# Westlake-AI/SemiReward

Measured on AMD Instinct MI355X. Metric: unlabeled images/sec/node (FlexMatch+SR, ViT-S CIFAR-100), higher is better.
Workload: dtype bf16

## Files before the change

include/srhip.h:

```cpp
#ifndef SRHIP_H
#define SRHIP_H

#ifdef __cplusplus
extern "C" {
#endif

enum {
  SRHIP_EPI_BF16 = 0,
  SRHIP_EPI_GELU_BF16 = 1,
  SRHIP_EPI_RESID_F32 = 2,
  SRHIP_EPI_DGELU_BF16 = 3,
  SRHIP_EPI_F32 = 4
};
int srhip_gemm_nt(int epilogue, const void* A, int lda, const void* B, int ldb, void* C, int ldc, int M, int N, int K,
                  const float* bias, const float* row_scale, int rows_per_sample, const void* aux_in, void* aux_out,
                  int ldaux, float alpha, float beta, void* stream);
#define SRHIP_GEMM_PLAN_TILE128 0
#define SRHIP_GEMM_PLAN_SMALL64 1
#define SRHIP_GEMM_PLAN_BIG256 2
#define SRHIP_GEMM_PLAN_BIG128 3
#define SRHIP_GEMM_PLAN_BIG2WG 4
#define SRHIP_GEMM_PLAN_PP256 5
int srhip_gemm_nt_plan(int epilogue, int M, int N, int K, float beta);
int srhip_gemm_nt_planned(int epilogue, const void* A, int lda, const void* B, int ldb, void* C, int ldc, int M, int N, int K,
// ... 32 lines not shown
} srhip_slab_desc;
int srhip_slab_reduce_f32(const srhip_slab_desc* desc_dev, int n, int total_blocks, void* stream);
int srhip_gemm_tn_grouped_pp_f32(const srhip_group_tn_desc* desc_dev, int n_problems, int total_tiles, float alpha, float beta,
                                 void* stream);

int srhip_attn_fwd(const void* qkv, void* out, float* lse, int B, int N, int H, float scale, void* stream);
int srhip_attn_bwd(const void* qkv, const void* out, const void* d_out, const float* lse, void* dqkv, float* delta_ws,
                   int B, int N, int H, float scale, void* stream);

int srhip_attn_masked_fwd(const void* qkv, void* out, float* lse, const int* key_len, int B, int N, int H, float scale,
                          unsigned drop_key, unsigned drop_thresh, float drop_scale, void* stream);
int srhip_attn_masked_bwd(const void* qkv, const void* out, const void* d_out, const float* lse, void* dqkv, float* delta_ws,
                          const int* key_len, int B, int N, int H, float scale, unsigned drop_key, unsigned drop_thresh,
                          float drop_scale, void* stream);

int srhip_layernorm_fwd(const float* x, const float* gamma, const float* beta, float eps, void* out, float* mean,
                        float* rstd, int M, int D, void* stream);
int srhip_layernorm_bwd(const void* dy, const float* x, const float* mean, const float* rstd, const float* gamma,
                        float* dx, float* dgamma, float* dbeta, int M, int D, void* stream);
int srhip_layernorm_bwd_cast(const void* dy, const float* x, const float* mean, const float* rstd, const float* gamma, float* dx, float* dgamma,
                             float* dbeta, void* out_bf16, const float* row_scale, int rows_per_sample, int M, int D, void* stream);
int srhip_layernorm_bwd_part(const void* dy, const float* x, const float* mean, const float* rstd, const float* gamma, float* dx, float* part,
                             int n_rep, void* out_bf16, const float* row_scale, int rows_per_sample, int M, int D, void* stream);
typedef struct srhip_ln_reduce_desc { float* dgamma; float* dbeta; } srhip_ln_reduce_desc;
int srhip_ln_grad_reduce(const srhip_ln_reduce_desc* desc_dev, float* part, int n_ln, int n_rep, int D, void* stream);
typedef struct srhip_dw_tail {
  const srhip_ln_reduce_desc* ln_desc; float* ln_part;
  const float* dlogits; const float* feat; float* dWh; float* dbh;
  const float* dx; const float* img; const int* img_index; float* dpos; float* dcls; float* pe_ws;
  int n_ln, n_rep, C, B, D, in_chans, HW, ps;
} srhip_dw_tail;
int srhip_gemm_tn_grouped_tail_f32(const srhip_group_tn_desc* desc_dev, int n_problems, int total_tiles, float alpha, float beta,
                                   const srhip_dw_tail* tail, void* stream);
int srhip_patch_embed_bwd_fold(const float* ws, float* dWp, float* dbp, int B, int C, int HW, int ps, int D, void* stream);

int srhip_mlp_fused(const float* x, float* x_out, const float* ln_gamma, const float* ln_beta, float eps, const void* W1,
                    const float* b1, const void* W2, const float* b2, const float* row_scale, int rows_per_sample, int save_rows,
                    void* save_ln2, void* save_pre, void* save_h, float* save_mean, float* save_rstd, int M, int D, int Hd,
                    void* stream);
int srhip_gelu_eval(const float* x, float* y_erf, float* y_poly, int n, void* stream);
int srhip_mlp_fused_proj(const float* x, float* x_out, const void* ao, const void* Wp, const float* bp, const float* row_scale1,
                         int ao_scaled, const float* ln_gamma, const float* ln_beta, float eps, const void* W1, const float* b1, const void* W2,
                         const float* b2, const float* row_scale2, int rows_per_sample, void* ln_next, const float* next_gamma,
                         const float* next_beta, int M, int D, int Hd, void* stream);
int srhip_mlp_fused_proj_strided(const float* x, float* x_out, const void* ao, const void* Wp, const float* bp, const float* row_scale1,
                                 int ao_scaled, const float* ln_gamma, const float* ln_beta, float eps, const void* W1, const float* b1,
                                 const void* W2, const float* b2, const float* row_scale2, int rows_per_sample, void* ln_next,
                                 const float* next_gamma, const float* next_beta, int M, int D, int Hd, int row_pitch, void* stream);

int srhip_attn_block_supported(int N, int D, int H);
int srhip_attn_block_fused(const void* xn_bf16, const void* Wqkv, const float* bqkv, const void* qkv_extra, void* out, const float* out_scale,
                           int B, int N, int D, int H, float scale, void* stream);

int srhip_patch_embed_fwd(const float* img, const int* img_index, const float* Wp, const float* bp, const float* cls,
                          const float* pos, float* x, int B, int C, int HW, int ps, int D, void* stream);
int srhip_patch_embed_bwd(const float* dx, const float* img, const int* img_index, float* dWp, float* dbp, float* dcls,
                          float* dpos, int B, int C, int HW, int ps, int D, void* stream);
long srhip_patch_embed_bwd_ws_floats(int B, int C, int HW, int ps, int D);
int srhip_patch_embed_bwd_ws(const float* dx, const float* img, const int* img_index, float* dWp, float* dbp, float* dcls,
                             float* dpos, float* ws, int B, int C, int HW, int ps, int D, void* stream);

int srhip_patch_im2col(const float* img, const int* img_index, void* out, int B, int C, int HW, int ps, void* stream);
int srhip_patch_assemble(const float* tok, const float* bp, const float* cls, const float* pos, float* x, int B, int Np, int D,
                         void* stream);
int srhip_patch_grad_operands(const float* dx, void* dx_tok_bf16, float* dpos, float* dcls, int B, int Np, int D, void* stream);

// ... 284 lines not shown
```

semireward_amd/_lib.py:

```python
import ctypes
import os
from ctypes import c_double, c_float, c_int, c_long, c_longlong, c_uint, c_ulonglong, c_void_p

import torch

HERE = os.path.dirname(os.path.abspath(__file__))
LIB_PATH = os.path.join(HERE, "libsrhip.so")

EPI_BF16, EPI_GELU_BF16, EPI_RESID_F32, EPI_DGELU_BF16, EPI_F32 = range(5)
X3_EPI_F32, X3_EPI_GELU_F32, X3_EPI_RESID_F32 = range(3)
X3B_NT, X3B_NN = range(2)
X3B_EPI_F32, X3B_EPI_ACC, X3B_EPI_DGELU, X3B_EPI_GELU_PRE = range(4)
REDUCE_NONE, REDUCE_MEAN, REDUCE_SUM = range(3)
SCORE_FIXED, SCORE_FLEX, SCORE_FREE, SCORE_SOFT = range(4)

P, I, F, L, Dbl, U = c_void_p, c_int, c_float, c_long, c_double, c_uint
SIGNATURES = {
    "srhip_gemm_nt": (I, [I, P, I, P, I, P, I, I, I, I, P, P, I, P, P, I, F, F, P]),
    "srhip_gemm_nt_plan": (I, [I, I, I, I, F]),
    "srhip_gemm_nt_planned": (I, [I, P, I, P, I, P, I, I, I, I, P, P, I, P, P, I, F, F, I, P]),
    "srhip_vit_fork": (I, [P, P, P, I, I, I, I, P]),
    "srhip_vit_fanout": (I, [P, P, I, P, P, I, P, P, c_longlong, I, I, P]),
    "srhip_gemm_small_max_grid": (I, [I]),
    "srhip_gemm_nt_grouped_f32": (I, [P, I, I, F, F, P]),
    "srhip_gemm_nt_grouped_n64_f32": (I, [P, I, I, F, F, P]),
    "srhip_gemm_tn_grouped_f32": (I, [P, I, I, F, F, P]),
    "srhip_gemm_tn_grouped_pp_f32": (I, [P, I, I, F, F, P]),
    "srhip_gemm_tn_grouped_tail_f32": (I, [P, I, I, F, F, P, P]),
    "srhip_patch_embed_bwd_fold": (I, [P, P, P, I, I, I, I, I, P]),
    "srhip_slab_reduce_f32": (I, [P, I, I, P]),
    "srhip_attn_fwd": (I, [P, P, P, I, I, I, F, P]),
    "srhip_attn_bwd": (I, [P, P, P, P, P, P, I, I, I, F, P]),
    "srhip_layernorm_fwd": (I, [P, P, P, F, P, P, P, I, I, P]),
    "srhip_layernorm_bwd": (I, [P, P, P, P, P, P, P, P, I, I, P]),
    "srhip_layernorm_bwd_cast": (I, [P, P, P, P, P, P, P, P, P, P, I, I, I, P]),
    "srhip_layernorm_bwd_part": (I, [P, P, P, P, P, P, P, I, P, P, I, I, I, P]),
    "srhip_ln_grad_reduce": (I, [P, P, I, I, I, P]),
    "srhip_mlp_fused": (I, [P, P, P, P, F, P, P, P, P, P, I, I, P, P, P, P, P, I, I, I, P]),
    "srhip_attn_block_supported": (I, [I, I, I]),
    "srhip_attn_block_fused": (I, [P, P, P, P, P, P, I, I, I, I, F, P]),
    "srhip_gelu_eval": (I, [P, P, P, I, P]),
    "srhip_mlp_fused_proj": (I, [P, P, P, P, P, P, I, P, P, F, P, P, P, P, P, I, P, P, P, I, I, I, P]),
    "srhip_mlp_fused_proj_strided": (I, [P, P, P, P, P, P, I, P, P, F, P, P, P, P, P, I, P, P, P, I, I, I, I, P]),
    "srhip_adam_bias_corrections": (I, [F, F, I, P]),
    "srhip_adamw_flat_dyn": (I, [P, P, P, P, P, P, P, I, P, P, P, F, F, F, Dbl, F, P, I, P]),
    "srhip_adam_flat_dyn": (I, [P, P, P, P, L, F, F, F, F, P, P]),
    "srhip_droppath_fill_cols_dyn": (I, [P, P, P, I, I, I, P, c_ulonglong, P]),
    "srhip_patch_embed_fwd": (I, [P, P, P, P, P, P, P, I, I, I, I, I, P]),
    "srhip_patch_embed_bwd": (I, [P, P, P, P, P, P, P, I, I, I, I, I, P]),
    "srhip_patch_embed_bwd_ws_floats": (L, [I, I, I, I, I]),
    "srhip_patch_embed_bwd_ws": (I, [P, P, P, P, P, P, P, P, I, I, I, I, I, P]),
    "srhip_patch_im2col": (I, [P, P, P, I, I, I, I, P]),
    "srhip_patch_assemble": (I, [P, P, P, P, P, I, I, I, P]),
    "srhip_patch_grad_operands": (I, [P, P, P, P, I, I, I, P]),
    "srhip_gemm_nt_x3": (I, [I, P, I, P, I, P, I, I, I, I, P, P, I, P]),
    "srhip_attn_fwd_x3": (I, [P, P, I, I, I, F, P]),
    "srhip_layernorm_fwd_f32": (I, [P, P, P, F, P, P, P, I, I, P]),
    "srhip_patch_im2col_f32": (I, [P, P, P, I, I, I, I, P]),
    "srhip_attn_fwd_x3_lse": (I, [P, P, P, I, I, I, F, P]),
    "srhip_gemm_x3": (I, [I, I, P, I, P, I, P, I, I, I, I, P, P, P, I, P]),
    "srhip_gemm_tn_x3_grouped": (I, [P, I, I, P]),
# ... 149 lines not shown
```

semireward_amd/csrc/gemm_tn.hip:

```cpp
#include <stdlib.h>

#include <type_traits>
#include <utility>

#include "../../include/srhip.h"
#include "common.h"
#include "tail_ops.h"

namespace {

constexpr int BM = 128, BN = 128, BK = 32;
constexpr int TILE = BK * BM;
constexpr int STAGE = 2 * TILE;
constexpr int NS = 3, PD = NS - 1;

typedef __attribute__((address_space(3))) void lds_void;
#define WAIT_VM(n) asm volatile("s_waitcnt vmcnt(" #n ")" ::: "memory")

typedef __attribute__((ext_vector_type(4))) short s16x4_t;
typedef __attribute__((address_space(3))) s16x4_t lds_s16x4;
__device__ __forceinline__ u32x2_t ds_read_tr16(const bf16_t* p) {
  return __builtin_bit_cast(u32x2_t, __builtin_amdgcn_ds_read_tr16_b64_v4i16((lds_s16x4*)p));
}

// ... 94 lines not shown
#pragma unroll
    for (int nt = 0; nt < 4; ++nt) {
      const int n = n0 + wn * 64 + nt * 16 + lg * 4;
      if (n >= d.N) continue;
      f32x4_t* cp = reinterpret_cast<f32x4_t*>(d.C + (size_t)m * d.ldc + n);
      f32x4_t x = {alpha * acc[nt][mt][0], alpha * acc[nt][mt][1], alpha * acc[nt][mt][2], alpha * acc[nt][mt][3]};
      if (atomic) {
        float* cf = d.C + (size_t)m * d.ldc + n;
        unsafeAtomicAdd(cf, x[0]); unsafeAtomicAdd(cf + 1, x[1]); unsafeAtomicAdd(cf + 2, x[2]); unsafeAtomicAdd(cf + 3, x[3]);
        continue;
      }
      if (beta != 0.0f && !overwrite) {
        const f32x4_t c = *cp;
        x[0] += beta * c[0]; x[1] += beta * c[1]; x[2] += beta * c[2]; x[3] += beta * c[3];
      }
      *cp = x;
    }
  }
}

__global__ __launch_bounds__(256, 3) void gemm_tn_grouped_f32_kernel(const srhip_group_tn_desc* __restrict__ desc, int n_problems,
                                                                     float alpha, float beta) {
  __shared__ __attribute__((aligned(16))) bf16_t smem[NS * STAGE];
  gemm_tn_tile_body(desc, n_problems, alpha, beta, xcd_remap(blockIdx.x, gridDim.x), smem);
}

__global__ __launch_bounds__(256, 3) void gemm_tn_grouped_tail_f32_kernel(const srhip_group_tn_desc* __restrict__ desc, int n_problems,
                                                                          int gemm_tiles, float alpha, float beta, const srhip_dw_tail t) {
  __shared__ __attribute__((aligned(16))) bf16_t smem[NS * STAGE];
  if ((int)blockIdx.x < gemm_tiles) {
    gemm_tn_tile_body(desc, n_problems, alpha, beta, xcd_remap(blockIdx.x, gemm_tiles), smem);
    return;
  }
  int b = blockIdx.x - gemm_tiles;
  const int tid = threadIdx.x;
  const int nlx = (2 * t.D + 255) / 256, nln = nlx * t.n_ln;
  if (b < nln) { ln_grad_reduce_body(t.ln_desc, t.ln_part, t.n_rep, t.D, b % nlx, b / nlx, tid); return; }
  b -= nln;
  if (b < t.C) { cls_head_bwd_w_body(t.dlogits, t.feat, t.dWh, t.dbh, t.B, t.D, t.C, b, tid); return; }
  b -= t.C;
  if (!t.dx) return;
  const int gw = t.HW / t.ps, N = gw * gw + 1, nch = (N - 1 + PE_TOK - 1) / PE_TOK;
  if (b < N) { pe_bwd_pos_body(t.dx, t.dpos, t.dcls, t.B, N, t.D, b, tid, 256); return; }
  b -= N;
  if (b < nch * t.B)
    pe_bwd_part_body(t.dx, t.img, t.img_index, t.pe_ws, t.in_chans, t.HW, t.ps, t.D, reinterpret_cast<float*>(smem), b % nch, b / nch, nch, tid, 256);
}


constexpr int PBK = 64;
constexpr int PH_EL = PBK * 128;
constexpr int PSLOT = 10;
constexpr int PLEAD = PSLOT - 2;
constexpr int PINFL = 2 * (PLEAD - 2);
constexpr int PGROUP_M = 8;

template <int N_>
__device__ __forceinline__ void wait_vm_n() { asm volatile("s_waitcnt vmcnt(%0)" ::"n"(N_) : "memory"); }

__device__ __forceinline__ void pp_tile_mn(int t, int ntm, int ntn, int& tm, int& tn) {
  const int band = t / (PGROUP_M * ntn), r = t - band * PGROUP_M * ntn;
  const int rows = min(PGROUP_M, ntm - band * PGROUP_M);
  tm = band * PGROUP_M + r % rows;
  tn = r / rows;
}

__global__ __launch_bounds__(512, 1) void gemm_tn_pp_kernel(const srhip_group_tn_desc* __restrict__ desc, int n_problems, int total_tiles,
                                                            float alpha, float beta) {
  extern __shared__ __attribute__((aligned(16))) bf16_t psm[];
  const int tid = threadIdx.x, lane = tid & 63;
  const int wave = __builtin_amdgcn_readfirstlane(tid >> 6);
  const int wr = wave >> 2, wc = wave & 3;
  const int l15 = lane & 15, lg = lane >> 4;
  const int first = xcd_remap(blockIdx.x, gridDim.x);
  if (first >= total_tiles) return;
  const int my_tiles = (total_tiles - first + gridDim.x - 1) / gridDim.x;

  const int prow = 4 * wave + (lane >> 4);
  const int pls = ((lane & 15) - 2 * prow) & 15;
// ... 235 lines not shown
    for (int s_ = 0; s_ < d.n_slabs; ++s_) {
      const f32x4_t v = *reinterpret_cast<const f32x4_t*>(d.src + (size_t)s_ * d.stride + i);
      a[0] += v[0]; a[1] += v[1]; a[2] += v[2]; a[3] += v[3];
    }
    *reinterpret_cast<f32x4_t*>(d.dst + i) = a;
  } else {
    for (int j = i; j < min(i + 4, d.count); ++j) {
      float a = d.dst[j];
      for (int s_ = 0; s_ < d.n_slabs; ++s_) a += d.src[(size_t)s_ * d.stride + j];
      d.dst[j] = a;
    }
  }
}

}

extern "C" int srhip_slab_reduce_f32(const srhip_slab_desc* desc_dev, int n, int total_blocks, void* stream) {
  if (!desc_dev || n <= 0 || total_blocks <= 0) return SR_EINVAL;
  SR_LAUNCH(slab_reduce_kernel, dim3(total_blocks), dim3(256), 0, (hipStream_t)stream, desc_dev, n);
  SR_CHECK_LAUNCH();
  return SR_OK;
}

extern "C" int srhip_gemm_tn_grouped_pp_f32(const srhip_group_tn_desc* desc_dev, int n_problems, int total_tiles, float alpha,
                                            float beta, void* stream) {
  if (!desc_dev || n_problems <= 0 || n_problems > 4096 || total_tiles <= 0) return SR_EINVAL;
  constexpr size_t sm = (size_t)PSLOT * PH_EL * sizeof(bf16_t);
  (void)hipFuncSetAttribute((const void*)gemm_tn_pp_kernel, hipFuncAttributeMaxDynamicSharedMemorySize, (int)sm);
  SR_LAUNCH(gemm_tn_pp_kernel, dim3(min(total_tiles, 256)), dim3(512), sm, (hipStream_t)stream, desc_dev, n_problems, total_tiles, alpha, beta);
  SR_CHECK_LAUNCH();
  return SR_OK;
}

extern "C" int srhip_gemm_tn_grouped_tail_f32(const srhip_group_tn_desc* desc_dev, int n_problems, int total_tiles, float alpha, float beta,
                                              const srhip_dw_tail* tail, void* stream) {
  if (!desc_dev || n_problems <= 0 || n_problems > 4096 || total_tiles <= 0 || !tail) return SR_EINVAL;
  const srhip_dw_tail t = *tail;
  if (t.D <= 0 || t.n_ln < 0 || t.C < 0 || (t.n_ln > 0 && (!t.ln_desc || !t.ln_part || t.n_rep <= 0))) return SR_EINVAL;
  if (t.C > 0 && (t.B <= 0 || !t.dlogits || !t.feat || !t.dWh || !t.dbh)) return SR_EINVAL;
  long extra = (long)cdiv(2 * t.D, 256) * t.n_ln + t.C;
  if (t.dx) {
    if (t.B <= 0 || t.in_chans <= 0 || t.ps <= 0 || t.HW <= 0 || t.HW % t.ps != 0 || t.D % 64 != 0 || t.D > 1024 ||
        t.in_chans * t.ps * t.ps > 64 || !t.img || !t.dpos || !t.dcls || !t.pe_ws)
      return SR_EINVAL;
    const int gw = t.HW / t.ps, N = gw * gw + 1;
    extra += N + (long)cdiv(N - 1, PE_TOK) * t.B;
  }
  if (total_tiles + extra > 0x7fffffffL) return SR_EINVAL;
  SR_LAUNCH(gemm_tn_grouped_tail_f32_kernel, dim3((unsigned)(total_tiles + extra)), dim3(256), 0, (hipStream_t)stream, desc_dev, n_problems,
                     total_tiles, alpha, beta, t);
  SR_CHECK_LAUNCH();
  return SR_OK;
}

extern "C" int srhip_gemm_tn_grouped_f32(const srhip_group_tn_desc* desc_dev, int n_problems, int total_tiles, float alpha,
                                         float beta, void* stream) {
  if (!desc_dev || n_problems <= 0 || n_problems > 4096 || total_tiles <= 0) return SR_EINVAL;
  SR_LAUNCH(gemm_tn_grouped_f32_kernel, dim3(total_tiles), dim3(256), 0, (hipStream_t)stream, desc_dev, n_problems, alpha,
                     beta);
  SR_CHECK_LAUNCH();
  return SR_OK;
}
```

semireward_amd/csrc/tail_ops.h:

```cpp
#pragma once
#include "common.h"
#include "srhip.h"

namespace {

constexpr int PE_TOK = 32;

__device__ __forceinline__ void ln_grad_reduce_body(const srhip_ln_reduce_desc* __restrict__ desc, float* __restrict__ part, int n_rep, int D,
                                                    int bx, int by, int tid) {
  const int c = bx * 256 + tid;
  if (c >= 2 * D) return;
  float* p = part + (size_t)by * n_rep * 2 * D + c;
  float acc = 0.f;
  for (int r = 0; r < n_rep; ++r) { acc += p[(size_t)r * 2 * D]; p[(size_t)r * 2 * D] = 0.f; }
  const srhip_ln_reduce_desc d = desc[by];
  float* dst = c < D ? d.dgamma + c : d.dbeta + (c - D);
  *dst += acc;
}

__device__ __forceinline__ void cls_head_bwd_w_body(const float* __restrict__ dlogits, const float* __restrict__ feat, float* __restrict__ dWh,
                                                    float* __restrict__ dbh, int B, int D, int C, int c, int tid) {
  for (int d = tid; d < D; d += 256) {
    float a = 0.f;
    for (int b = 0; b < B; ++b) a += dlogits[(size_t)b * C + c] * feat[(size_t)b * D + d];
// ... 29 lines not shown
    const int c = k / (ps * ps), i = (k / ps) % ps, j = k % ps;
    patch[e] = im[((size_t)c * HW + py * ps + i) * HW + px * ps + j];
  }
  __syncthreads();
  for (int d = tid; d < D; d += nthr) {
    const float* g0 = dx + ((size_t)b * N + t0) * D + d;
    float* out = ws + (size_t)(by * nbx + bx) * (K + 1) * D + d;
    float accb = 0.f;
    for (int k0 = 0; k0 < K; k0 += 16) {
      float acc[16];
#pragma unroll
      for (int k = 0; k < 16; ++k) acc[k] = 0.f;
      for (int tb = 0; tb < nt; tb += 8) {
        float g[8];
#pragma unroll
        for (int i = 0; i < 8; ++i) g[i] = (tb + i < nt) ? g0[(size_t)(tb + i) * D] : 0.f;
#pragma unroll
        for (int i = 0; i < 8; ++i) {
          const int tt = min(tb + i, nt - 1);
          if (k0 == 0) accb += g[i];
#pragma unroll
          for (int k = 0; k < 16; ++k)
            if (k0 + k < K) acc[k] += g[i] * patch[tt * K + k0 + k];
        }
      }
#pragma unroll
      for (int k = 0; k < 16; ++k)
        if (k0 + k < K) out[(size_t)(k0 + k) * D] = acc[k];
    }
    out[(size_t)K * D] = accb;
  }
}

}
```

semireward_amd/nets/vit.py:

```python
import math
import types

import numpy as np
import torch

from .. import ops
from .pretrained import load_checkpoint
from .surface import ModuleSurface


class VitConfig:
    def __init__(self, img_size=224, patch_size=16, in_chans=3, num_classes=1000, embed_dim=768, depth=12,
                 num_heads=12, mlp_ratio=4.0, drop_path_rate=0.0, eps=1e-6):
        self.img_size, self.patch_size, self.in_chans, self.num_classes = img_size, patch_size, in_chans, num_classes
        self.embed_dim, self.depth, self.num_heads, self.mlp_ratio = embed_dim, depth, num_heads, mlp_ratio
        self.drop_path_rate, self.eps = drop_path_rate, eps
        assert embed_dim % num_heads == 0 and embed_dim // num_heads == 64, "libsrhip attention is built for head_dim 64"
        assert embed_dim in (128, 384, 768)

    @property
    def num_tokens(self):
        return (self.img_size // self.patch_size) ** 2 + 1

    @property
    def hidden(self):
        return int(self.embed_dim * self.mlp_ratio)


def param_names_shapes(cfg):
    D, Hd, p, C = cfg.embed_dim, cfg.hidden, cfg.patch_size, cfg.num_classes
    out = [("cls_token", (1, 1, D)), ("pos_embed", (1, cfg.num_tokens, D)),
           ("patch_embed.proj.weight", (D, cfg.in_chans, p, p)), ("patch_embed.proj.bias", (D,))]
    for i in range(cfg.depth):
        b = "blocks.%d." % i
        out += [(b + "norm1.weight", (D,)), (b + "norm1.bias", (D,)),
                (b + "attn.qkv.weight", (3 * D, D)), (b + "attn.qkv.bias", (3 * D,)),
                (b + "attn.proj.weight", (D, D)), (b + "attn.proj.bias", (D,)),
                (b + "norm2.weight", (D,)), (b + "norm2.bias", (D,)),
                (b + "mlp.fc1.weight", (Hd, D)), (b + "mlp.fc1.bias", (Hd,)),
                (b + "mlp.fc2.weight", (D, Hd)), (b + "mlp.fc2.bias", (D,))]
    out += [("norm.weight", (D,)), ("norm.bias", (D,)), ("head.weight", (C, D)), ("head.bias", (C,))]
    return out


DW_GROUPS = 3
LN_REP = 16
_FUSED_MLP = True
_FUSED_ATTN = True
_FUSED_PROJ = True
_FUSED_NEXT_LN = True
_LAST_BLOCK_CLASS_ROWS = True
_FUSED_MLP_MIN_ROWS = 16384


def _fused_mlp(cfg, rows):
    Hd = cfg.hidden
    return cfg.embed_dim == 384 and Hd % 128 == 0 and Hd <= 4096 and rows >= _FUSED_MLP_MIN_ROWS and _FUSED_MLP


def launch_kernels(cfg, n_images, kernels_as_images=None, precision="bf16"):
    if precision == "bf16x3":
        return ("bf16x3",)
    D, N, H, Hd = cfg.embed_dim, cfg.num_tokens, cfg.num_heads, cfg.hidden
    M = n_images * N
    fused = _fused_mlp(cfg, max(M, (kernels_as_images or 0) * N))
    fused_attn = _FUSED_ATTN and ops.attn_block_supported(N, D, H)
    gemms = []
    if cfg.in_chans * cfg.patch_size ** 2 > 64:
        gemms.append((ops.EPI_F32, n_images * (N - 1), D, cfg.in_chans * cfg.patch_size ** 2))
    if not fused_attn:
        gemms.append((ops.EPI_BF16, M, 3 * D, D))
    if not (fused and _FUSED_PROJ):
        gemms.append((ops.EPI_RESID_F32, M, D, D))
    if not fused:
        gemms += [(ops.EPI_GELU_BF16, M, Hd, D), (ops.EPI_RESID_F32, M, D, Hd)]
    return (fused, fused_attn) + tuple(ops.gemm_nt_plan(e, m, n, k) for e, m, n, k in gemms)


def droppath_keep_host(probs, depth, B, seed, cols=None):
    p = np.asarray(probs, dtype=np.float32)[:depth]
    col = np.arange(B, dtype=np.int64) if cols is None else np.asarray(cols, dtype=np.int64)
    col = np.where((col < 0) | (col >= B), 0, col)
    i = (np.arange(2 * depth, dtype=np.int64)[:, None] * B + col[None, :]).astype(np.uint64)
    with np.errstate(over="ignore"):
# ... 285 lines not shown
            ops.gemm_nt_x3(ops.X3_EPI_F32, ln, P(b + "attn.qkv.weight"), qkv, M, 3 * D, D, bias=P(b + "attn.qkv.bias"))
            if save:
                ops.attn_fwd_x3_lse(qkv, ao, ctx.lse[i], B, N, H, scale)
                xm = ctx.xmid[i]
                xm.copy_(x)
            else:
                ops.attn_fwd_x3(qkv, ao, B, N, H, scale)
                xm = x
            ops.gemm_nt_x3(ops.X3_EPI_RESID_F32, ao, P(b + "attn.proj.weight"), xm, M, D, D, bias=P(b + "attn.proj.bias"),
                           row_scale=s1, rows_per_sample=N)
            ops.layernorm_fwd_f32(xm, P(b + "norm2.weight"), P(b + "norm2.bias"), cfg.eps, ln2, st2[0], st2[1], M, D)
            if save:
                ops.gemm_x3(ops.X3B_NT, ops.X3B_EPI_GELU_PRE, ln2, P(b + "mlp.fc1.weight"), hbuf, M, Hd, D, bias=P(b + "mlp.fc1.bias"),
                            aux_out=ctx.pre[i], ldaux=Hd)
                xn = ctx.xs[i + 1]
                xn.copy_(xm)
            else:
                ops.gemm_nt_x3(ops.X3_EPI_GELU_F32, ln2, P(b + "mlp.fc1.weight"), hbuf, M, Hd, D, bias=P(b + "mlp.fc1.bias"))
                xn = xm
            ops.gemm_nt_x3(ops.X3_EPI_RESID_F32, hbuf, P(b + "mlp.fc2.weight"), xn, M, D, Hd, bias=P(b + "mlp.fc2.bias"),
                           row_scale=s2, rows_per_sample=N)
            x = xn
        return self._head(x, B, out, ctx, tree, tag)

    def forward(self, x, only_fc=False, only_feat=False, **kw):
        assert not only_fc, "only_fc is not on the SemiReward hot path"
        dp = self.make_droppath(x.shape[0]) if (self.training and self.cfg.drop_path_rate > 0) else None
        logits, feat, _ = self.forward_features(x.contiguous(), None, dp, save=False)
        return feat if only_feat else {"logits": logits, "feat": feat}

    __call__ = forward

    def _bwd_plan(self, M, ctx):
        key = ("bwdplan", M, id(ctx))
        if key in self._buf_cache:
            return self._buf_cache[key]
        cfg = self.cfg
        D, Hd = cfg.embed_dim, cfg.hidden
        x3 = ctx.precision == "bf16x3"
        make_desc = ops.make_group_tn_x3_desc if x3 else ops.make_group_tn_desc
        mk = lambda c: torch.empty(M, c, dtype=torch.float32 if x3 else torch.bfloat16, device=self.device)
        layers, problems = [], []
        G = lambda n: self.view(n, self.grad)
        for i in range(cfg.depth):
            b = "blocks.%d." % i
            t = dict(g2=mk(D), dpre=mk(Hd), g1=mk(D), dqkv=mk(3 * D))
            layers.append(t)
            problems += [(t["g2"], ctx.h[i], G(b + "mlp.fc2.weight"), G(b + "mlp.fc2.bias"), D, Hd, M),
                         (t["dpre"], ctx.ln2[i], G(b + "mlp.fc1.weight"), G(b + "mlp.fc1.bias"), Hd, D, M),
                         (t["g1"], ctx.ao[i], G(b + "attn.proj.weight"), G(b + "attn.proj.bias"), D, D, M),
                         (t["dqkv"], ctx.ln1[i], G(b + "attn.qkv.weight"), G(b + "attn.qkv.bias"), 3 * D, D, M)]
        out = dict(layers=layers, desc=make_desc(problems, self.device))
        ln_names = lambda lo_l, hi_l: [(G("blocks.%d.norm%d.weight" % (i, j)), G("blocks.%d.norm%d.bias" % (i, j)))
                                       for i in range(lo_l, hi_l) for j in (1, 2)]
        out["ln_part"] = torch.zeros(2 * cfg.depth, LN_REP, 2, D, dtype=torch.float32, device=self.device)
        out["ln_desc"] = ops.make_ln_reduce_desc(ln_names(0, cfg.depth), self.device)

        def flat_range(lo_l, hi_l):
            names = [n for n, _ in self.names_shapes if n.startswith("blocks.") and lo_l <= int(n.split(".")[1]) < hi_l]
            lo = min(self.offsets[n][0] for n in names)
            hi = max(self.offsets[n][0] + int(torch.Size(self.offsets[n][1]).numel()) for n in names)
            assert sum(int(torch.Size(self.offsets[n][1]).numel()) for n in names) == hi - lo, "block parameters are contiguous in the flat block"
            return lo, hi
        out["flat"] = flat_range(0, cfg.depth)
        groups = []
        if not x3:
            ng = max(1, min(DW_GROUPS, cfg.depth))
            per = -(-cfg.depth // ng)
            for hi_l in range(cfg.depth, 0, -per):
                lo_l = max(0, hi_l - per)
                groups.append(dict(lo_layer=lo_l, hi_layer=hi_l, flat=flat_range(lo_l, hi_l),
                                   desc=make_desc(problems[4 * lo_l:4 * hi_l], self.device),
                                   ln_desc=ops.make_ln_reduce_desc(ln_names(lo_l, hi_l), self.device)))
        out["groups"] = groups
        self._buf_cache[key] = out
        return out

    def backward(self, ctx, dlogits):
        self.backward_rows(ctx, dlogits, 0, ctx.B)
        self.backward_finish(ctx, dlogits)

    def _bwd_views(self, ctx, T, b0, b1):
        key = ("bwdviews", id(ctx), b0, b1)
        v = self._buf_cache.get(key)
        if v is not None:
            return v
        cfg = self.cfg
        D, N, H = cfg.embed_dim, cfg.num_tokens, cfg.num_heads
# ... 166 lines not shown
```

semireward_amd/ops.py:

```python
import ctypes
import os

import torch

from . import _lib
from ._lib import EPI_BF16, EPI_DGELU_BF16, EPI_F32, EPI_GELU_BF16, EPI_RESID_F32
from ._lib import X3_EPI_F32, X3_EPI_GELU_F32, X3_EPI_RESID_F32
from ._lib import X3B_NT, X3B_NN, X3B_EPI_F32, X3B_EPI_ACC, X3B_EPI_DGELU, X3B_EPI_GELU_PRE
from ._lib import REDUCE_NONE, REDUCE_MEAN, REDUCE_SUM


_CHECK_ARGS = os.environ.get("SRHIP_CHECK_ARGS", "0") != "0"


def _p_checked(t):
    if t is None:
        return None
    assert t.is_cuda and t.is_contiguous(), "libsrhip needs contiguous device tensors"
    return t.data_ptr()


def _p_fast(t):
    return None if t is None else t.data_ptr()

# ... 233 lines not shown


class TableStager:

    def __init__(self, nbytes, depth=8):
        self.bufs = [torch.empty(nbytes, dtype=torch.uint8).pin_memory() for _ in range(depth)]
        self.events = [None] * depth
        self.i = 0

    def upload(self, arr_u8, device):
        n = int(arr_u8.size)
        slot = self.i % len(self.bufs)
        self.i += 1
        if n > self.bufs[slot].numel():
            return torch.from_numpy(arr_u8.copy()).to(device)
        if self.events[slot] is not None:
            self.events[slot].synchronize()
        self.bufs[slot][:n].copy_(torch.from_numpy(arr_u8))
        dev = torch.empty(n, dtype=torch.uint8, device=device)
        dev.copy_(self.bufs[slot][:n], non_blocking=True)
        ev = torch.cuda.Event()
        ev.record()
        self.events[slot] = ev
        return dev


SLAB_DESC_DTYPE = [("dst", "<u8"), ("src", "<u8"), ("stride", "<i8"), ("count", "<i4"), ("n_slabs", "<i4"), ("block_start", "<i4"), ("pad0", "<i4")]
TN_OVERWRITE = 2


def make_group_tn_desc(problems, device, split_k=0, tile=128, slabs=False, stager=None):
    import numpy as np
    assert all(pr[6] > 0 and pr[4] % 8 == 0 and pr[5] % 8 == 0 for pr in problems), "K >= 1 tokens; M, N multiples of 8 (srhip.h)"
    plan = [(tuple(pr), split_k if (split_k > 0 and pr[6] >= 2 * split_k) else 0) for pr in problems]
    if tile == 256 and split_k == 0:
        plan = tn_pp_plan(problems)
    slabs = slabs and any(sk > 0 for _, sk in plan)
    lay, n_el = [], 0
    if slabs:
        for (A, B, C, db, M, N, K), sk in plan:
            if sk > 0:
                nsl = -(-K // sk)
                oc = n_el
                n_el += nsl * M * N
                ob = n_el
                n_el += nsl * M if db is not None else 0
                n_el = -(-n_el // 4) * 4
                lay.append((oc, ob, nsl))
            else:
                lay.append(None)
        slab = torch.empty(max(n_el, 4), dtype=torch.float32, device=device)
    ent, red = [], []
    t = rb = 0
    for i, ((A, B, C, db, M, N, K), sk) in enumerate(plan):
        tiles = ((M + tile - 1) // tile) * ((N + tile - 1) // tile)
        if sk > 0:
            for si, k0 in enumerate(range(0, K, sk)):
                if slabs:
                    oc, ob, nsl = lay[i]
                    cp = slab.data_ptr() + 4 * (oc + si * M * N)
                    bp = slab.data_ptr() + 4 * (ob + si * M) if db is not None else 0
                    ent.append((_p(A) + 2 * k0 * M, _p(B) + 2 * k0 * N, cp, bp, M, N, min(sk, K - k0), M, N, N, t, TN_OVERWRITE))
                else:
                    ent.append((_p(A) + 2 * k0 * M, _p(B) + 2 * k0 * N, _p(C), _p(db) or 0, M, N, min(sk, K - k0), M, N, N, t, TN_ATOMIC))
                t += tiles
            if slabs:
                oc, ob, nsl = lay[i]
                red.append((_p(C), slab.data_ptr() + 4 * oc, M * N, M * N, nsl, rb, 0))
                rb += -(-M * N // 1024)
                if db is not None:
                    red.append((_p(db), slab.data_ptr() + 4 * ob, M, M, nsl, rb, 0))
                    rb += -(-M // 1024)
        else:
            ent.append((_p(A), _p(B), _p(C), _p(db) or 0, M, N, K, M, N, N, t, 0))
            t += tiles
    arr = np.zeros(len(ent), dtype=GROUP_TN_DESC_DTYPE)
    for i, e in enumerate(ent):
        arr[i] = e
    assert arr.itemsize == 64
    flops = float(sum(2.0 * M * N * K for *_, M, N, K in problems))
    nbytes = float(sum(2.0 * (M * K + N * K) + 8.0 * M * N for *_, M, N, K in problems))
    up = (lambda a: stager.upload(a.view(np.uint8).reshape(-1), device)) if stager is not None else (lambda a: torch.from_numpy(a.view(np.uint8).copy()).to(device))
    desc = up(arr)
    desc.out_ranges = [(e[2], 4 * e[4] * e[5]) for e in ent] + [(e[3], 4 * e[4]) for e in ent if e[3]]
    if slabs:
        ra = np.zeros(len(red), dtype=SLAB_DESC_DTYPE)
        for i, e in enumerate(red):
            ra[i] = e
        assert ra.itemsize == 40
        desc.slab = slab
        desc.reduce = (up(ra), len(red), rb)
    return desc, len(ent), t, flops, nbytes


TN_PP_GRID = 256


def tn_pp_plan(problems, grid=TN_PP_GRID):
    tiles = [((M + 255) // 256) * ((N + 255) // 256) for *_, M, N, K in problems]
    total = sum(tiles)
    rem = total % grid
    plan = [(tuple(pr), 0) for pr in problems]
    if total < grid or rem == 0 or rem > 0.7 * grid:
        return plan
    got = 0
    for i in range(len(problems) - 1, -1, -1):
        if got >= rem:
            break
        K = problems[i][6]
        want = max(2, min(8, grid // max(rem, 1)))
        n = min(want, K // 512)
        if n >= 2:
            sl = -(-K // n)
            sl = -(-sl // 64) * 64
            plan[i] = (tuple(problems[i]), sl)
        got += tiles[i]
    return plan


def tn_pp_efficiency(problems):
    area = sum(M * N for *_, M, N, K in problems)
    cover = sum(((M + 255) // 256) * ((N + 255) // 256) * 65536 for *_, M, N, K in problems)
    return area / max(cover, 1)


def gemm_tn_grouped_f32(desc, n_problems, total_tiles, alpha=1.0, beta=1.0, flops=0.0, nbytes=0.0, pp=False):
    fn, kern = ("srhip_gemm_tn_grouped_pp_f32", "gemm_tn_pp_kernel") if pp else ("srhip_gemm_tn_grouped_f32", "gemm_tn_grouped_f32_kernel")
    red = getattr(desc, "reduce", None)
    if red is not None:
        assert beta == 1.0, "a table with slab slices is a C += product"
    if _PROFILE is not None:
        _PROFILE.timed(fn, (_p(desc), n_problems, total_tiles, alpha, beta, _s(),), flops, kern, nbytes)
    else:
        _call(fn, _p(desc), n_problems, total_tiles, alpha, beta, _s())
    if red is not None:
        _call("srhip_slab_reduce_f32", _p(red[0]), red[1], red[2], _s())


def gemm_tn_grouped_tail_f32(desc, n_problems, total_tiles, D, ln=None, head=None, pe=None, alpha=1.0, beta=1.0):
    from ._lib import DwTail
    assert getattr(desc, "reduce", None) is None, "a table with slab slices has a second phase of its own"
    t = DwTail()
    t.D = D
    if ln is not None:
        t.ln_desc, t.ln_part, t.n_ln, t.n_rep = _p(ln[0]), _p(ln[1]), ln[2], ln[3]
    if head is not None:
        t.dlogits, t.feat, t.dWh, t.dbh, t.B, t.C = _p(head[0]), _p(head[1]), _p(head[2]), _p(head[3]), head[4], head[5]
    if pe is not None:
        assert head is None or head[4] == pe[6]
        t.dx, t.img, t.img_index, t.dpos, t.dcls, t.pe_ws = (_p(x) for x in pe[:6])
        t.B, t.in_chans, t.HW, t.ps = pe[6:]
    if _CHECK_ARGS:
        mine = list(getattr(ln[0], "out_ranges", ())) if ln is not None else []
        mine += [(_p(x), x.numel() * x.element_size()) for x in ((head[2], head[3]) if head is not None else ()) + (tuple(pe[3:6]) if pe is not None else ())]
        for a0, an in mine:
            for b0, bn in getattr(desc, "out_ranges", ()):
                assert a0 + an <= b0 or b0 + bn <= a0, "a tail output of gemm_tn_grouped_tail_f32 overlaps a C / dbias of the table"
    _call("srhip_gemm_tn_grouped_tail_f32", _p(desc), n_problems, total_tiles, alpha, beta, ctypes.addressof(t), _s())


def attn_block_supported(N, D, H):
    from ._lib import lib
    return bool(lib().srhip_attn_block_supported(N, D, H))


def attn_block_fused(xn, Wqkv, bqkv, out, B, N, D, H, scale, qkv_extra=None, out_scale=None):
    if N == 257:
        gemm_nt(EPI_BF16, xn[256:], Wqkv, qkv_extra, B, 3 * D, D, lda=N * D, bias=bqkv)
    if _PROFILE is not None:
        M = B * N
        _PROFILE.timed("srhip_attn_block_fused", (_p(xn), _p(Wqkv), _p(bqkv), _p(qkv_extra), _p(out), _p(out_scale), B, N, D, H, scale, _s(),), 2.0 * M * 3 * D * D + 4.0 * B * H * N * N * 64, "attn_block_kernel<%d>" % N,
                              2.0 * M * D + 2.0 * M * D + 2.0 * 3 * D * D)
        return
    _call("srhip_attn_block_fused", _p(xn), _p(Wqkv), _p(bqkv), _p(qkv_extra), _p(out), _p(out_scale), B, N, D, H, scale, _s())


def attn_fwd(qkv, out, lse, B, N, H, scale):
    if _PROFILE is not None:
        _PROFILE.timed("srhip_attn_fwd", (_p(qkv), _p(out), _p(lse), B, N, H, scale, _s()), 4.0 * B * H * N * N * 64, "attn_fwd_kernel",
                       2.0 * B * N * 4 * H * 64)
        return
    _call("srhip_attn_fwd", _p(qkv), _p(out), _p(lse), B, N, H, scale, _s())


def attn_bwd(qkv, out, d_out, lse, dqkv, delta_ws, B, N, H, scale):
    if _PROFILE is not None:
        _PROFILE.timed("srhip_attn_bwd", (_p(qkv), _p(out), _p(d_out), _p(lse), _p(dqkv), _p(delta_ws), B, N, H, scale, _s()),
                       10.0 * B * H * N * N * 64, "attn_bwd (dq + dkv kernels)", 2.0 * B * N * 8 * H * 64)
        return
    _call("srhip_attn_bwd", _p(qkv), _p(out), _p(d_out), _p(lse), _p(dqkv), _p(delta_ws), B, N, H, scale, _s())

# ... 960 lines not shown
```

Measured before the change: 1624.

## Add 128x384 tile variant of grouped TN weight-gradient GEMM for ViT-S

```diff
diff --git a/include/srhip.h b/include/srhip.h
--- a/include/srhip.h
+++ b/include/srhip.h
@@ -88,6 +88,10 @@
 } srhip_dw_tail;
 int srhip_gemm_tn_grouped_tail_f32(const srhip_group_tn_desc* desc_dev, int n_problems, int total_tiles, float alpha, float beta,
                                    const srhip_dw_tail* tail, void* stream);
+int srhip_gemm_tn_grouped_w384_f32(const srhip_group_tn_desc* desc_dev, const srhip_group_tn_desc* desc_host, int n_problems, int total_tiles,
+                                   float alpha, float beta, void* stream);
+int srhip_gemm_tn_grouped_tail_w384_f32(const srhip_group_tn_desc* desc_dev, const srhip_group_tn_desc* desc_host, int n_problems,
+                                        int total_tiles, float alpha, float beta, const srhip_dw_tail* tail, void* stream);
 int srhip_patch_embed_bwd_fold(const float* ws, float* dWp, float* dbp, int B, int C, int HW, int ps, int D, void* stream);
 
 int srhip_mlp_fused(const float* x, float* x_out, const float* ln_gamma, const float* ln_beta, float eps, const void* W1,
diff --git a/semireward_amd/_lib.py b/semireward_amd/_lib.py
--- a/semireward_amd/_lib.py
+++ b/semireward_amd/_lib.py
@@ -27,6 +27,8 @@
     "srhip_gemm_tn_grouped_f32": (I, [P, I, I, F, F, P]),
     "srhip_gemm_tn_grouped_pp_f32": (I, [P, I, I, F, F, P]),
     "srhip_gemm_tn_grouped_tail_f32": (I, [P, I, I, F, F, P, P]),
+    "srhip_gemm_tn_grouped_w384_f32": (I, [P, P, I, I, F, F, P]),
+    "srhip_gemm_tn_grouped_tail_w384_f32": (I, [P, P, I, I, F, F, P, P]),
     "srhip_patch_embed_bwd_fold": (I, [P, P, P, I, I, I, I, I, P]),
     "srhip_slab_reduce_f32": (I, [P, I, I, P]),
     "srhip_attn_fwd": (I, [P, P, P, I, I, I, F, P]),
diff --git a/semireward_amd/csrc/gemm_tn.hip b/semireward_amd/csrc/gemm_tn.hip
--- a/semireward_amd/csrc/gemm_tn.hip
+++ b/semireward_amd/csrc/gemm_tn.hip
@@ -150,19 +150,141 @@
     gemm_tn_tile_body(desc, n_problems, alpha, beta, xcd_remap(blockIdx.x, gemm_tiles), smem);
     return;
   }
-  int b = blockIdx.x - gemm_tiles;
-  const int tid = threadIdx.x;
-  const int nlx = (2 * t.D + 255) / 256, nln = nlx * t.n_ln;
-  if (b < nln) { ln_grad_reduce_body(t.ln_desc, t.ln_part, t.n_rep, t.D, b % nlx, b / nlx, tid); return; }
-  b -= nln;
-  if (b < t.C) { cls_head_bwd_w_body(t.dlogits, t.feat, t.dWh, t.dbh, t.B, t.D, t.C, b, tid); return; }
-  b -= t.C;
-  if (!t.dx) return;
-  const int gw = t.HW / t.ps, N = gw * gw + 1, nch = (N - 1 + PE_TOK - 1) / PE_TOK;
-  if (b < N) { pe_bwd_pos_body(t.dx, t.dpos, t.dcls, t.B, N, t.D, b, tid, 256); return; }
-  b -= N;
-  if (b < nch * t.B)
-    pe_bwd_part_body(t.dx, t.img, t.img_index, t.pe_ws, t.in_chans, t.HW, t.ps, t.D, reinterpret_cast<float*>(smem), b % nch, b / nch, nch, tid, 256);
+  dw_tail_body(t, blockIdx.x - gemm_tiles, threadIdx.x, reinterpret_cast<float*>(smem));
+}
+
+constexpr int WBN = 384, WPIECES = WBN / BN, WNT = WBN / 32;
+constexpr int WSTAGE = (1 + WPIECES) * TILE;
+constexpr int WNS = 2;
+
+__device__ __forceinline__ void gemm_tn_tile_body_w384(const srhip_group_tn_desc* __restrict__ desc, int n_problems, float alpha, float beta,
+                                                       const int tile, bf16_t* smem) {
+  int p = 0;
+  {
+    int lo = 0, hi = n_problems - 1;
+    while (lo < hi) { const int mid = (lo + hi + 1) >> 1; if (tile >= desc[mid].tile_start) lo = mid; else hi = mid - 1; }
+    p = lo;
+  }
+  const srhip_group_tn_desc d = desc[p];
+  const int local = tile - d.tile_start, ntn = d.N / WBN;
+  const int m0 = (local / ntn) * BM, n0 = (local % ntn) * WBN;
+  const int tid = threadIdx.x, lane = tid & 63;
+  const int wave = __builtin_amdgcn_readfirstlane(tid >> 6);
+  const int wm = wave >> 1, wn = wave & 1;
+  const int l15 = lane & 15, lg = lane >> 4;
+  const int nk = (d.K + BK - 1) / BK;
+
+  const __amdgpu_buffer_rsrc_t ra = __builtin_amdgcn_make_buffer_rsrc(const_cast<void*>(d.A), 0, max(d.K * d.lda, (d.K - 1) * d.lda + d.M) * 2, 0x00020000);
+  const __amdgpu_buffer_rsrc_t rb = __builtin_amdgcn_make_buffer_rsrc(const_cast<void*>(d.B), 0, max(d.K * d.ldb, (d.K - 1) * d.ldb + d.N) * 2, 0x00020000);
+  int va[2], vb[2];
+#pragma unroll
+  for (int i = 0; i < 2; ++i) {
+    const int row = 8 * wave + 4 * i + (lane >> 4);
+    const int ch = ((lane & 15) - 2 * row) & 15;
+    va[i] = (row * d.lda + 8 * ch) * 2;
+    vb[i] = (row * d.ldb + 8 * ch) * 2;
+  }
+  const int sa0 = m0 * 2, sb0 = n0 * 2, sak = BK * d.lda * 2, sbk = BK * d.ldb * 2;
+#define ISSUE_W(kt_, st_)                                                                                                \
+  _Pragma("unroll") for (int i = 0; i < 2; ++i) {                                                                        \
+    bf16_t* da = smem + (st_) * WSTAGE + (8 * wave + 4 * i) * BM;                                                        \
+    __builtin_amdgcn_raw_ptr_buffer_load_lds(ra, (lds_void*)da, 16, va[i], sa0 + (kt_) * sak, 0, 0);                      \
+    _Pragma("unroll") for (int j = 0; j < WPIECES; ++j)                                                                  \
+      __builtin_amdgcn_raw_ptr_buffer_load_lds(rb, (lds_void*)(da + (1 + j) * TILE), 16, vb[i], sb0 + 2 * BN * j + (kt_) * sbk, 0, 0); \
+  }
+
+  const int r0 = 4 * lg + (l15 >> 2);
+  int fo_a[WNT], fo_b[4];
+#pragma unroll
+  for (int t = 0; t < WNT; ++t) {
+    const int cn = wn * (WBN / 2) + t * 16 + 4 * (l15 & 3), c0 = cn & (BN - 1);
+    fo_a[t] = (1 + (cn >> 7)) * TILE + r0 * BM + ((((c0 >> 3) + 2 * r0) & 15) << 3) + (c0 & 4);
+  }
+#pragma unroll
+  for (int t = 0; t < 4; ++t) {
+    const int cm = wm * 64 + t * 16 + 4 * (l15 & 3);
+    fo_b[t] = r0 * BM + ((((cm >> 3) + 2 * r0) & 15) << 3) + (cm & 4);
+  }
+  f32x4_t acc[WNT][4], accb[4];
+#pragma unroll
+  for (int i = 0; i < 4; ++i) accb[i] = f32x4_t{0.f, 0.f, 0.f, 0.f};
+#pragma unroll
+  for (int i = 0; i < WNT; ++i)
+#pragma unroll
+    for (int j = 0; j < 4; ++j) acc[i][j] = f32x4_t{0.f, 0.f, 0.f, 0.f};
+  const bool want_bias = d.dbias != nullptr && n0 == 0 && wn == 0;
+  const u32x4_t ones = u32x4_t{0x3f803f80u, 0x3f803f80u, 0x3f803f80u, 0x3f803f80u};
+
+  if (nk > 0) { ISSUE_W(0, 0) }
+  for (int kt = 0; kt < nk; ++kt) {
+    WAIT_VM(0);
+    __builtin_amdgcn_s_barrier();
+    if (kt + 1 < nk) { ISSUE_W(kt + 1, (kt + 1) & 1) }
+    const bf16_t* st = smem + (kt & 1) * WSTAGE;
+    u32x4_t fb[4];
+#pragma unroll
+    for (int t = 0; t < 4; ++t) {
+      const u32x2_t b0 = ds_read_tr16(st + fo_b[t]), b1 = ds_read_tr16(st + fo_b[t] + 16 * BM);
+      fb[t] = u32x4_t{b0[0], b0[1], b1[0], b1[1]};
+    }
+    if (want_bias) {
+#pragma unroll
+      for (int mt = 0; mt < 4; ++mt)
+        accb[mt] = __builtin_amdgcn_mfma_f32_16x16x32_bf16(__builtin_bit_cast(bf16x8_t, ones), __builtin_bit_cast(bf16x8_t, fb[mt]),
+                                                           accb[mt], 0, 0, 0);
+    }
+#pragma unroll
+    for (int nt = 0; nt < WNT; ++nt) {
+      const u32x2_t a0 = ds_read_tr16(st + fo_a[nt]), a1 = ds_read_tr16(st + fo_a[nt] + 16 * BM);
+      const u32x4_t fa = u32x4_t{a0[0], a0[1], a1[0], a1[1]};
+#pragma unroll
+      for (int mt = 0; mt < 4; ++mt)
+        acc[nt][mt] = __builtin_amdgcn_mfma_f32_16x16x32_bf16(__builtin_bit_cast(bf16x8_t, fa), __builtin_bit_cast(bf16x8_t, fb[mt]),
+                                                              acc[nt][mt], 0, 0, 0);
+    }
+  }
+#undef ISSUE_W
+
+  const bool atomic = (d.flags & SRHIP_TN_ATOMIC) != 0;
+  const bool overwrite = (d.flags & SRHIP_TN_OVERWRITE) != 0;
+#pragma unroll
+  for (int mt = 0; mt < 4; ++mt) {
+    const int m = m0 + wm * 64 + mt * 16 + l15;
+    if (m >= d.M) continue;
+    if (want_bias && lg == 0) {
+      if (atomic) unsafeAtomicAdd(d.dbias + m, accb[mt][0]); else if (overwrite) d.dbias[m] = accb[mt][0]; else d.dbias[m] += accb[mt][0];
+    }
+#pragma unroll
+    for (int nt = 0; nt < WNT; ++nt) {
+      float* cf = d.C + (size_t)m * d.ldc + n0 + wn * (WBN / 2) + nt * 16 + lg * 4;
+      f32x4_t x = {alpha * acc[nt][mt][0], alpha * acc[nt][mt][1], alpha * acc[nt][mt][2], alpha * acc[nt][mt][3]};
+      if (atomic) {
+        unsafeAtomicAdd(cf, x[0]); unsafeAtomicAdd(cf + 1, x[1]); unsafeAtomicAdd(cf + 2, x[2]); unsafeAtomicAdd(cf + 3, x[3]);
+        continue;
+      }
+      if (beta != 0.0f && !overwrite) {
+        const f32x4_t c = *reinterpret_cast<const f32x4_t*>(cf);
+        x[0] += beta * c[0]; x[1] += beta * c[1]; x[2] += beta * c[2]; x[3] += beta * c[3];
+      }
+      *reinterpret_cast<f32x4_t*>(cf) = x;
+    }
+  }
+}
+
+__global__ __launch_bounds__(256, 2) void gemm_tn_grouped_w384_f32_kernel(const srhip_group_tn_desc* __restrict__ desc, int n_problems,
+                                                                          float alpha, float beta) {
+  __shared__ __attribute__((aligned(16))) bf16_t smem[WNS * WSTAGE];
+  gemm_tn_tile_body_w384(desc, n_problems, alpha, beta, xcd_remap(blockIdx.x, gridDim.x), smem);
+}
+
+__global__ __launch_bounds__(256, 2) void gemm_tn_grouped_tail_w384_f32_kernel(const srhip_group_tn_desc* __restrict__ desc, int n_problems,
+                                                                               int gemm_tiles, float alpha, float beta, const srhip_dw_tail t) {
+  __shared__ __attribute__((aligned(16))) bf16_t smem[WNS * WSTAGE];
+  if ((int)blockIdx.x < gemm_tiles) {
+    gemm_tn_tile_body_w384(desc, n_problems, alpha, beta, xcd_remap(blockIdx.x, gemm_tiles), smem);
+    return;
+  }
+  dw_tail_body(t, blockIdx.x - gemm_tiles, threadIdx.x, reinterpret_cast<float*>(smem));
 }
 
 
@@ -464,23 +586,62 @@
   return SR_OK;
 }
 
+static long dw_tail_extra(const srhip_dw_tail& t) {
+  if (t.D <= 0 || t.n_ln < 0 || t.C < 0 || (t.n_ln > 0 && (!t.ln_desc || !t.ln_part || t.n_rep <= 0))) return -1;
+  if (t.C > 0 && (t.B <= 0 || !t.dlogits || !t.feat || !t.dWh || !t.dbh)) return -1;
+  long extra = (long)cdiv(2 * t.D, 256) * t.n_ln + t.C;
+  if (t.dx) {
+    if (t.B <= 0 || t.in_chans <= 0 || t.ps <= 0 || t.HW <= 0 || t.HW % t.ps != 0 || t.D % 64 != 0 || t.D > 1024 ||
+        t.in_chans * t.ps * t.ps > 64 || !t.img || !t.dpos || !t.dcls || !t.pe_ws)
+      return -1;
+    const int gw = t.HW / t.ps, N = gw * gw + 1;
+    extra += N + (long)cdiv(N - 1, PE_TOK) * t.B;
+  }
+  return extra;
+}
+
 extern "C" int srhip_gemm_tn_grouped_tail_f32(const srhip_group_tn_desc* desc_dev, int n_problems, int total_tiles, float alpha, float beta,
                                               const srhip_dw_tail* tail, void* stream) {
   if (!desc_dev || n_problems <= 0 || n_problems > 4096 || total_tiles <= 0 || !tail) return SR_EINVAL;
   const srhip_dw_tail t = *tail;
-  if (t.D <= 0 || t.n_ln < 0 || t.C < 0 || (t.n_ln > 0 && (!t.ln_desc || !t.ln_part || t.n_rep <= 0))) return SR_EINVAL;
-  if (t.C > 0 && (t.B <= 0 || !t.dlogits || !t.feat || !t.dWh || !t.dbh)) return SR_EINVAL;
-  long extra = (long)cdiv(2 * t.D, 256) * t.n_ln + t.C;
-  if (t.dx) {
-    if (t.B <= 0 || t.in_chans <= 0 || t.ps <= 0 || t.HW <= 0 || t.HW % t.ps != 0 || t.D % 64 != 0 || t.D > 1024 ||
-        t.in_chans * t.ps * t.ps > 64 || !t.img || !t.dpos || !t.dcls || !t.pe_ws)
-      return SR_EINVAL;
-    const int gw = t.HW / t.ps, N = gw * gw + 1;
-    extra += N + (long)cdiv(N - 1, PE_TOK) * t.B;
-  }
-  if (total_tiles + extra > 0x7fffffffL) return SR_EINVAL;
+  const long extra = dw_tail_extra(t);
+  if (extra < 0 || total_tiles + extra > 0x7fffffffL) return SR_EINVAL;
   SR_LAUNCH(gemm_tn_grouped_tail_f32_kernel, dim3((unsigned)(total_tiles + extra)), dim3(256), 0, (hipStream_t)stream, desc_dev, n_problems,
                      total_tiles, alpha, beta, t);
+  SR_CHECK_LAUNCH();
+  return SR_OK;
+}
+
+static bool w384_table_ok(const srhip_group_tn_desc* h, int n_problems, int total_tiles) {
+  long t = 0;
+  for (int i = 0; i < n_problems; ++i) {
+    const srhip_group_tn_desc& d = h[i];
+    if (!d.A || !d.B || !d.C || d.M <= 0 || d.N <= 0 || d.K <= 0 || d.N % WBN != 0 || d.M % 4 != 0 || d.tile_start != t) return false;
+    if (d.lda % 8 != 0 || d.ldb % 8 != 0 || d.ldc < d.N || d.ldc % 4 != 0) return false;
+    t += (long)cdiv(d.M, BM) * (d.N / WBN);
+    if (t > 0x7fffffffL) return false;
+  }
+  return t == total_tiles;
+}
+
+extern "C" int srhip_gemm_tn_grouped_w384_f32(const srhip_group_tn_desc* desc_dev, const srhip_group_tn_desc* desc_host, int n_problems,
+                                              int total_tiles, float alpha, float beta, void* stream) {
+  if (!desc_dev || !desc_host || n_problems <= 0 || n_problems > 4096 || total_tiles <= 0) return SR_EINVAL;
+  if (!w384_table_ok(desc_host, n_problems, total_tiles)) return SR_EINVAL;
+  SR_LAUNCH(gemm_tn_grouped_w384_f32_kernel, dim3(total_tiles), dim3(256), 0, (hipStream_t)stream, desc_dev, n_problems, alpha, beta);
+  SR_CHECK_LAUNCH();
+  return SR_OK;
+}
+
+extern "C" int srhip_gemm_tn_grouped_tail_w384_f32(const srhip_group_tn_desc* desc_dev, const srhip_group_tn_desc* desc_host, int n_problems,
+                                                   int total_tiles, float alpha, float beta, const srhip_dw_tail* tail, void* stream) {
+  if (!desc_dev || !desc_host || n_problems <= 0 || n_problems > 4096 || total_tiles <= 0 || !tail) return SR_EINVAL;
+  if (!w384_table_ok(desc_host, n_problems, total_tiles)) return SR_EINVAL;
+  const srhip_dw_tail t = *tail;
+  const long extra = dw_tail_extra(t);
+  if (extra < 0 || total_tiles + extra > 0x7fffffffL) return SR_EINVAL;
+  SR_LAUNCH(gemm_tn_grouped_tail_w384_f32_kernel, dim3((unsigned)(total_tiles + extra)), dim3(256), 0, (hipStream_t)stream, desc_dev,
+                     n_problems, total_tiles, alpha, beta, t);
   SR_CHECK_LAUNCH();
   return SR_OK;
 }
diff --git a/semireward_amd/csrc/tail_ops.h b/semireward_amd/csrc/tail_ops.h
--- a/semireward_amd/csrc/tail_ops.h
+++ b/semireward_amd/csrc/tail_ops.h
@@ -85,4 +85,17 @@
   }
 }
 
+__device__ __forceinline__ void dw_tail_body(const srhip_dw_tail& t, int b, int tid, float* lds) {
+  const int nlx = (2 * t.D + 255) / 256, nln = nlx * t.n_ln;
+  if (b < nln) { ln_grad_reduce_body(t.ln_desc, t.ln_part, t.n_rep, t.D, b % nlx, b / nlx, tid); return; }
+  b -= nln;
+  if (b < t.C) { cls_head_bwd_w_body(t.dlogits, t.feat, t.dWh, t.dbh, t.B, t.D, t.C, b, tid); return; }
+  b -= t.C;
+  if (!t.dx) return;
+  const int gw = t.HW / t.ps, N = gw * gw + 1, nch = (N - 1 + PE_TOK - 1) / PE_TOK;
+  if (b < N) { pe_bwd_pos_body(t.dx, t.dpos, t.dcls, t.B, N, t.D, b, tid, 256); return; }
+  b -= N;
+  if (b < nch * t.B) pe_bwd_part_body(t.dx, t.img, t.img_index, t.pe_ws, t.in_chans, t.HW, t.ps, t.D, lds, b % nch, b / nch, nch, tid, 256);
 }
+
+}
diff --git a/semireward_amd/nets/vit.py b/semireward_amd/nets/vit.py
--- a/semireward_amd/nets/vit.py
+++ b/semireward_amd/nets/vit.py
@@ -50,6 +50,7 @@
 _FUSED_PROJ = True
 _FUSED_NEXT_LN = True
 _LAST_BLOCK_CLASS_ROWS = True
+_DW_TILE_384 = True
 _FUSED_MLP_MIN_ROWS = 16384
 
 
@@ -401,28 +402,30 @@
     __call__ = forward
 
     def _bwd_plan(self, M, ctx):
-        key = ("bwdplan", M, id(ctx))
+        cfg = self.cfg
+        D, Hd = cfg.embed_dim, cfg.hidden
+        x3 = ctx.precision == "bf16x3"
+        w384 = _DW_TILE_384 and not x3 and D % 384 == 0 and Hd % 384 == 0
+        key = ("bwdplan", M, id(ctx), w384)
         if key in self._buf_cache:
             return self._buf_cache[key]
-        cfg = self.cfg
-        D, Hd = cfg.embed_dim, cfg.hidden
-        x3 = ctx.precision == "bf16x3"
+        other = self._buf_cache.get(("bwdplan", M, id(ctx), not w384))
         make_desc = ops.make_group_tn_x3_desc if x3 else ops.make_group_tn_desc
         mk = lambda c: torch.empty(M, c, dtype=torch.float32 if x3 else torch.bfloat16, device=self.device)
         layers, problems = [], []
         G = lambda n: self.view(n, self.grad)
         for i in range(cfg.depth):
             b = "blocks.%d." % i
-            t = dict(g2=mk(D), dpre=mk(Hd), g1=mk(D), dqkv=mk(3 * D))
+            t = other["layers"][i] if other is not None else dict(g2=mk(D), dpre=mk(Hd), g1=mk(D), dqkv=mk(3 * D))
             layers.append(t)
             problems += [(t["g2"], ctx.h[i], G(b + "mlp.fc2.weight"), G(b + "mlp.fc2.bias"), D, Hd, M),
                          (t["dpre"], ctx.ln2[i], G(b + "mlp.fc1.weight"), G(b + "mlp.fc1.bias"), Hd, D, M),
                          (t["g1"], ctx.ao[i], G(b + "attn.proj.weight"), G(b + "attn.proj.bias"), D, D, M),
                          (t["dqkv"], ctx.ln1[i], G(b + "attn.qkv.weight"), G(b + "attn.qkv.bias"), 3 * D, D, M)]
-        out = dict(layers=layers, desc=make_desc(problems, self.device))
+        out = dict(layers=layers, desc=make_desc(problems, self.device, tile=384) if w384 else make_desc(problems, self.device))
         ln_names = lambda lo_l, hi_l: [(G("blocks.%d.norm%d.weight" % (i, j)), G("blocks.%d.norm%d.bias" % (i, j)))
                                        for i in range(lo_l, hi_l) for j in (1, 2)]
-        out["ln_part"] = torch.zeros(2 * cfg.depth, LN_REP, 2, D, dtype=torch.float32, device=self.device)
+        out["ln_part"] = other["ln_part"] if other is not None else torch.zeros(2 * cfg.depth, LN_REP, 2, D, dtype=torch.float32, device=self.device)
         out["ln_desc"] = ops.make_ln_reduce_desc(ln_names(0, cfg.depth), self.device)
 
         def flat_range(lo_l, hi_l):
diff --git a/semireward_amd/ops.py b/semireward_amd/ops.py
--- a/semireward_amd/ops.py
+++ b/semireward_amd/ops.py
@@ -289,6 +289,9 @@
 def make_group_tn_desc(problems, device, split_k=0, tile=128, slabs=False, stager=None):
     import numpy as np
     assert all(pr[6] > 0 and pr[4] % 8 == 0 and pr[5] % 8 == 0 for pr in problems), "K >= 1 tokens; M, N multiples of 8 (srhip.h)"
+    assert tile in (128, 256, 384)
+    if tile == 384:
+        assert all(pr[5] % 384 == 0 for pr in problems) and not slabs, "128 x 384 tiles: every N a multiple of 384, no slab phase"
     plan = [(tuple(pr), split_k if (split_k > 0 and pr[6] >= 2 * split_k) else 0) for pr in problems]
     if tile == 256 and split_k == 0:
         plan = tn_pp_plan(problems)
@@ -310,7 +313,7 @@
     ent, red = [], []
     t = rb = 0
     for i, ((A, B, C, db, M, N, K), sk) in enumerate(plan):
-        tiles = ((M + tile - 1) // tile) * ((N + tile - 1) // tile)
+        tiles = ((M + 127) // 128) * (N // 384) if tile == 384 else ((M + tile - 1) // tile) * ((N + tile - 1) // tile)
         if sk > 0:
             for si, k0 in enumerate(range(0, K, sk)):
                 if slabs:
@@ -340,6 +343,9 @@
     up = (lambda a: stager.upload(a.view(np.uint8).reshape(-1), device)) if stager is not None else (lambda a: torch.from_numpy(a.view(np.uint8).copy()).to(device))
     desc = up(arr)
     desc.out_ranges = [(e[2], 4 * e[4] * e[5]) for e in ent] + [(e[3], 4 * e[4]) for e in ent if e[3]]
+    desc.tn_tile = tile
+    if tile == 384:
+        desc.host = arr
     if slabs:
         ra = np.zeros(len(red), dtype=SLAB_DESC_DTYPE)
         for i, e in enumerate(red):
@@ -383,13 +389,18 @@
 
 def gemm_tn_grouped_f32(desc, n_problems, total_tiles, alpha=1.0, beta=1.0, flops=0.0, nbytes=0.0, pp=False):
     fn, kern = ("srhip_gemm_tn_grouped_pp_f32", "gemm_tn_pp_kernel") if pp else ("srhip_gemm_tn_grouped_f32", "gemm_tn_grouped_f32_kernel")
+    tile = getattr(desc, "tn_tile", None)
+    assert tile is None or (tile == 256) == bool(pp), "the table counts other tiles than the kernel asked for"
+    head = (_p(desc),)
+    if tile == 384:
+        fn, kern, head = "srhip_gemm_tn_grouped_w384_f32", "gemm_tn_grouped_w384_f32_kernel", (_p(desc), desc.host.ctypes.data)
     red = getattr(desc, "reduce", None)
     if red is not None:
         assert beta == 1.0, "a table with slab slices is a C += product"
     if _PROFILE is not None:
-        _PROFILE.timed(fn, (_p(desc), n_problems, total_tiles, alpha, beta, _s(),), flops, kern, nbytes)
+        _PROFILE.timed(fn, head + (n_problems, total_tiles, alpha, beta, _s(),), flops, kern, nbytes)
     else:
-        _call(fn, _p(desc), n_problems, total_tiles, alpha, beta, _s())
+        _call(fn, *head, n_problems, total_tiles, alpha, beta, _s())
     if red is not None:
         _call("srhip_slab_reduce_f32", _p(red[0]), red[1], red[2], _s())
 
@@ -413,7 +424,10 @@
         for a0, an in mine:
             for b0, bn in getattr(desc, "out_ranges", ()):
                 assert a0 + an <= b0 or b0 + bn <= a0, "a tail output of gemm_tn_grouped_tail_f32 overlaps a C / dbias of the table"
-    _call("srhip_gemm_tn_grouped_tail_f32", _p(desc), n_problems, total_tiles, alpha, beta, ctypes.addressof(t), _s())
+    if getattr(desc, "tn_tile", 128) == 384:
+        _call("srhip_gemm_tn_grouped_tail_w384_f32", _p(desc), desc.host.ctypes.data, n_problems, total_tiles, alpha, beta, ctypes.addressof(t), _s())
+    else:
+        _call("srhip_gemm_tn_grouped_tail_f32", _p(desc), n_problems, total_tiles, alpha, beta, ctypes.addressof(t), _s())
 
 
 def attn_block_supported(N, D, H):
```

Result: no change. 1632 (median of 5 runs) (+0.5%).
